# danilodjor/fault-tolerant-llm-training

Measured on AMD Instinct MI355X. Metric: tokens/sec/GPU seq-len 2048 DP at 1/2/4/8 MI355X; checkpoint save wall-clock (s), higher is better.
Workload: dtype bf16; 1 GPU; model=llama3-8b, global_batch=1, seq_len=2048, parallelism=dp1

## Files before the change

csrc/kernels/embedding.hip:

```cpp
#include "torch_utils.h"

#include <algorithm>

namespace {

__global__ __launch_bounds__(256) void emb_fwd_kernel(const int64_t* __restrict__ tok,
                                                      const char* __restrict__ w,
                                                      char* __restrict__ out, int T, int row_bytes) {
  const int row = blockIdx.x;
  const int64_t t = tok[row];
  const uint4* src = reinterpret_cast<const uint4*>(w + t * (long)row_bytes);
  uint4* dst = reinterpret_cast<uint4*>(out + (long)row * row_bytes);
  for (int c = threadIdx.x; c < row_bytes / 16; c += blockDim.x) dst[c] = src[c];
}

constexpr int SORT_NT = 1024, SORT_W = SORT_NT / 64, SORT_BITS = 6, SORT_BINS = 1 << SORT_BITS;

__global__ __launch_bounds__(SORT_NT) void tok_sort_kernel(const int64_t* __restrict__ tok, int T, int passes,
                                                           int* __restrict__ keys, int* __restrict__ vals) {
  __shared__ int hist[SORT_BINS];
  __shared__ int start[SORT_BINS];
  __shared__ int rbase[SORT_BINS];
  __shared__ int wcnt[SORT_W][SORT_BINS];
  const int tid = threadIdx.x, lane = tid & 63, wid = tid >> 6;
// ... 96 lines not shown
                                                         float* __restrict__ part, int nparts) {
  __shared__ float red[4];
  const int lane = threadIdx.x & 63, wid = threadIdx.x >> 6;
  float sq = 0.f;
  for (int wave = blockIdx.x * 4 + wid; wave < T; wave += gridDim.x * 4) {
    const int t = sorted_tok[wave];
    if (wave > 0 && sorted_tok[wave - 1] == t) continue;
    int end = wave + 1;
    while (end < T && sorted_tok[end] == t) ++end;
    typename E::T* dst = dw + t * (long)D;
    for (int c = lane * 8; c < D; c += 64 * 8) {
      float acc[8] = {0, 0, 0, 0, 0, 0, 0, 0};
      for (int k = wave; k < end; ++k) {
        float x[8];
        ld8<E>(dy + perm[k] * (long)D + c, x);
#pragma unroll
        for (int j = 0; j < 8; ++j) acc[j] += x[j];
      }
      const P8<E> r = pk8<E>(acc);
      *reinterpret_cast<uint4*>(dst + c) = r.v[0];
      if constexpr (!E::is16) *reinterpret_cast<uint4*>(dst + c + 4) = r.v[1];
      float st[8];
      unp8<E>(r, st);
#pragma unroll
      for (int j = 0; j < 8; ++j) sq = fmaf(st[j], st[j], sq);
    }
  }
  const float tot = block_sum<256>(sq, red);
  if (threadIdx.x == 0) part[blockIdx.x] = tot;
  for (long i = blockIdx.x + (long)gridDim.x * (1 + threadIdx.x); i < nparts; i += (long)gridDim.x * 256)
    part[i] = 0.f;
}

}

at::Tensor embedding_fwd(const at::Tensor& tokens, const at::Tensor& weight) {
  FT_CHECK_CUDA(weight);
  FT_CHECK_MODEL_DTYPE(weight);
  FT_CHECK_CONTIG(weight);
  FT_CHECK_CONTIG(tokens);
  TORCH_CHECK(tokens.scalar_type() == at::kLong, "embedding: tokens must be int64");
  const int D = weight.size(1);
  TORCH_CHECK(D % 8 == 0, "embedding: dim must be a multiple of 8");
  const int T = tokens.numel();
  const at::DeviceGuard guard(weight.device());
  auto sizes = tokens.sizes().vec();
  sizes.push_back(D);
  auto out = at::empty(sizes, weight.options());
  if (T > 0)
    hipLaunchKernelGGL(emb_fwd_kernel, dim3(T), dim3(256), 0, ft_stream(), cptr<int64_t>(tokens),
                       cptr<char>(weight), mptr<char>(out), T, (int)(D * weight.element_size()));
  FT_LAUNCH_CHECK();
  return out;
}

void embedding_bwd_(const at::Tensor& dy, const at::Tensor& tokens, const at::Tensor& dw,
                    bool accumulate, const std::optional<at::Tensor>& part) {
  FT_CHECK_CUDA(dy);
  FT_CHECK_MODEL_DTYPE(dy);
  TORCH_CHECK(dy.scalar_type() == dw.scalar_type(), "embedding_bwd: dtype mismatch");
  FT_CHECK_CONTIG(dy);
  FT_CHECK_CONTIG(dw);
  const int D = dw.size(1);
  const int T = tokens.numel();
  TORCH_CHECK(dy.numel() == (long)T * D, "embedding_bwd: shape mismatch");
  const at::DeviceGuard guard(dw.device());
  TORCH_CHECK(tokens.scalar_type() == at::kLong, "embedding_bwd: tokens must be int64");
  const long V = dw.size(0);
  TORCH_CHECK(V >= 1 && V < (1L << 30), "embedding_bwd: vocabulary size out of range");
  int bits = 1;
  while ((1L << bits) < V) ++bits;
  const int passes = (bits + SORT_BITS - 1) / SORT_BITS;
  auto flat = tokens.reshape({-1}).contiguous();
  if (!accumulate) FT_HIP_CHECK(hipMemsetAsync(dw.data_ptr(), 0, dw.nbytes(), ft_stream()));
  if (T > 0) {
    auto kv = at::empty({4, (long)T}, tokens.options().dtype(at::kInt));
    int* keys = mptr<int>(kv);
    int* vals = keys + 2L * T;
    hipLaunchKernelGGL(tok_sort_kernel, dim3(1), dim3(SORT_NT), 0, ft_stream(), cptr<int64_t>(flat), T, passes,
                       keys, vals);
    FT_LAUNCH_CHECK();
    const long fin = (long)((passes - 1) & 1) * T;
    const int blocks = (T * 64 + 255) / 256;
    const bool sq = part.has_value() && part->defined();
    if (sq) {
      TORCH_CHECK(!accumulate, "embedding_bwd: norm partials need a fresh gradient");
      FT_CHECK_F32((*part));
      FT_CHECK_CONTIG((*part));
      const int np = (int)part->numel();
      const int g = std::max(1, std::min({blocks, 256, np}));
      FT_DISPATCH_E(dy.scalar_type(),
                    hipLaunchKernelGGL(emb_bwd_sq_kernel<E>, dim3(g), dim3(256), 0, ft_stream(), keys + fin,
                                       vals + fin, cptr<typename E::T>(dy), mptr<typename E::T>(dw), T, D,
                                       mptr<float>(*part), np));
    } else {
      FT_DISPATCH_E(dy.scalar_type(),
                    hipLaunchKernelGGL(emb_bwd_kernel<E>, dim3(blocks), dim3(256), 0, ft_stream(), keys + fin,
                                       vals + fin, cptr<typename E::T>(dy), mptr<typename E::T>(dw), T, D,
                                       accumulate));
    }
  } else if (part.has_value() && part->defined()) {
    part->zero_();
  }
  FT_LAUNCH_CHECK();
}

TORCH_LIBRARY_FRAGMENT(ftamd, m) {
  m.def("embedding_fwd(Tensor tokens, Tensor weight) -> Tensor", &embedding_fwd);
  m.def("embedding_bwd_(Tensor dy, Tensor tokens, Tensor(a!) dw, bool accumulate, Tensor(b!)? part=None) -> ()",
        &embedding_bwd_);
}
```

csrc/kernels/optim.hip:

```cpp
#include "torch_utils.h"

#include <vector>

#include <cstdlib>

namespace {

typedef unsigned int u32x4_t __attribute__((ext_vector_type(4)));

template <bool NT>
__device__ __forceinline__ uint4 ld16(const void* p) {
  if constexpr (NT) {
    const u32x4_t v = __builtin_nontemporal_load(reinterpret_cast<const u32x4_t*>(p));
    return make_uint4(v.x, v.y, v.z, v.w);
  } else {
    return *reinterpret_cast<const uint4*>(p);
  }
}

template <bool NT>
__device__ __forceinline__ void st16(void* p, uint4 v) {
  if constexpr (NT) {
    const u32x4_t w = {v.x, v.y, v.z, v.w};
    __builtin_nontemporal_store(w, reinterpret_cast<u32x4_t*>(p));
  } else {
    *reinterpret_cast<uint4*>(p) = v;
  }
}

template <class E, bool NT>
struct V8 {
  __device__ static void load(const typename E::T* p, float* f) {
    P8<E> r;
    r.v[0] = ld16<NT>(p);
    if constexpr (!E::is16) r.v[1] = ld16<NT>(p + 4);
    unp8<E>(r, f);
  }
  __device__ static void store(typename E::T* p, const float* f) {
    const P8<E> r = pk8<E>(f);
    st16<NT>(p, r.v[0]);
    if constexpr (!E::is16) st16<NT>(p + 4, r.v[1]);
  }
};

bool stream_nt() { return true; }

constexpr int NORM_BLOCKS = 2048;

template <class G, bool NT>
__global__ __launch_bounds__(256) void sumsq_kernel(const typename G::T* __restrict__ g, long n8,
                                                    float* __restrict__ partial) {
  float s = 0.f;
  for (long i = blockIdx.x * 256L + threadIdx.x; i < n8; i += (long)gridDim.x * 256) {
    float x[8];
    V8<G, NT>::load(g + i * 8, x);
#pragma unroll
    for (int j = 0; j < 8; ++j) s += x[j] * x[j];
  }
  __shared__ float red[4];
  s = block_sum<256>(s, red);
  if (threadIdx.x == 0) partial[blockIdx.x] = s;
}

__global__ __launch_bounds__(1024) void norm_finish_kernel(const float* __restrict__ partial,
                                                           int np, float extra_sumsq_scale,
                                                           float max_norm,
                                                           float* __restrict__ stats) {
  float s = 0.f;
  const int n4 = np >> 2;
  const float4* p4 = reinterpret_cast<const float4*>(partial);
  if ((reinterpret_cast<uintptr_t>(partial) & 15) == 0) {
    for (int i = threadIdx.x; i < n4; i += 1024) {
      const float4 v = p4[i];
      s += (v.x + v.y) + (v.z + v.w);
    }
    for (int i = 4 * n4 + threadIdx.x; i < np; i += 1024) s += partial[i];
  } else {
    for (int i = threadIdx.x; i < np; i += 1024) s += partial[i];
  }
  __shared__ float red[16];
  s = block_sum<1024>(s, red);
  if (threadIdx.x == 0) {
    const float norm = sqrtf(s * extra_sumsq_scale);
    stats[0] = norm;
    const bool bad = !isfinite(norm);
    stats[1] = (max_norm > 0.f && !bad) ? fminf(1.f, max_norm / (norm + 1e-6f)) : 1.f;
    stats[2] = (bad || stats[2] != 0.f) ? 1.f : 0.f;
  }
}

template <class P, class S, bool NT>
__global__ __launch_bounds__(256) void adamw_kernel(typename P::T* __restrict__ p,
                                                    const typename P::T* __restrict__ g,
                                                    typename S::T* __restrict__ m,
                                                    typename S::T* __restrict__ v,
                                                    long n8, float lr, float beta1, float beta2,
                                                    float eps, float wd, float inv_bc1,
                                                    float inv_sqrt_bc2,
                                                    const float* __restrict__ stats,
                                                    const float* __restrict__ hyper, int exact) {
  if (stats[2] != 0.f) return;
  if (hyper != nullptr) {
    lr = hyper[0];
    inv_bc1 = hyper[1];
    inv_sqrt_bc2 = hyper[2];
  }
  const float coef = stats[1];
  const float decay = 1.f - lr * wd;
  const float step = lr * inv_bc1;
  for (long i = blockIdx.x * 256L + threadIdx.x; i < n8; i += (long)gridDim.x * 256) {
    float pf[8], gf[8], mf[8], vf[8];
    V8<P, NT>::load(p + i * 8, pf);
    V8<P, NT>::load(g + i * 8, gf);
    V8<S, NT>::load(m + i * 8, mf);
    V8<S, NT>::load(v + i * 8, vf);
#pragma unroll
    for (int j = 0; j < 8; ++j) {
      const float gj = gf[j] * coef;
      pf[j] *= decay;
      mf[j] += (gj - mf[j]) * (1.f - beta1);
      vf[j] = vf[j] * beta2 + (1.f - beta2) * gj * gj;
      if (exact) {
        const float denom = sqrtf(vf[j]) * inv_sqrt_bc2 + eps;
        pf[j] -= step * mf[j] / denom;
      } else {
        const float denom = fast_sqrt(vf[j]) * inv_sqrt_bc2 + eps;
        pf[j] -= step * mf[j] * fast_rcp(denom);
      }
    }
    V8<P, NT>::store(p + i * 8, pf);
    V8<S, NT>::store(m + i * 8, mf);
    V8<S, NT>::store(v + i * 8, vf);
  }
}

int stream_grid(long n8) {
  long g = (n8 + 255) / 256;
  return (int)std::max(1L, std::min(g, 65535L));
}

void launch_sumsq(const at::Tensor& grad, long n8, int nb, float* partial) {
  const bool nt = stream_nt();
  FT_DISPATCH_E(grad.scalar_type(), {
    if (nt)
      hipLaunchKernelGGL((sumsq_kernel<E, true>), dim3(nb), dim3(256), 0, ft_stream(),
                         cptr<typename E::T>(grad), n8, partial);
    else
      hipLaunchKernelGGL((sumsq_kernel<E, false>), dim3(nb), dim3(256), 0, ft_stream(),
                         cptr<typename E::T>(grad), n8, partial);
  });
}

}

void grad_norm_(const at::Tensor& grad, const at::Tensor& stats, double max_norm) {
  FT_CHECK_CUDA(grad);
  FT_CHECK_CONTIG(grad);
  FT_CHECK_F32(stats);
  TORCH_CHECK(grad.numel() % 8 == 0, "grad_norm: numel must be a multiple of 8");
  const at::DeviceGuard guard(grad.device());
  const long n8 = grad.numel() / 8;
  const int nb = std::max(1, std::min(NORM_BLOCKS, (int)((n8 + 255) / 256)));
  auto partial = at::empty({nb}, grad.options().dtype(at::kFloat));
  launch_sumsq(grad, n8, nb, mptr<float>(partial));
  FT_LAUNCH_CHECK();
  hipLaunchKernelGGL(norm_finish_kernel, dim3(1), dim3(1024), 0, ft_stream(), cptr<float>(partial), nb,
// ... 26 lines not shown
  const float bc1 = 1.f - (float)std::pow(beta1, (double)step);
  const float bc2 = 1.f - (float)std::pow(beta2, (double)step);
  const float inv_bc1 = 1.f / bc1, inv_sqrt_bc2 = 1.f / std::sqrt(bc2);
  int nb = stream_grid(n8);
  if (max_blocks > 0) nb = (int)std::max(1L, std::min((n8 + 255) / 256, (long)max_blocks));
  const dim3 grid(nb), block(256);
  const bool nt = stream_nt();
  TORCH_CHECK(m.scalar_type() == p.scalar_type() || m.scalar_type() == at::kFloat,
              "adamw: optimizer states must have the parameter dtype or fp32");
  const int exact = (int)ft_exact_math() || p.scalar_type() == at::kFloat;
  auto go = [&](auto ptag, auto stag) {
    using P = decltype(ptag);
    using S = decltype(stag);
    using PT = typename P::T;
    using ST = typename S::T;
    if (nt)
      hipLaunchKernelGGL((adamw_kernel<P, S, true>), grid, block, 0, ft_stream(), mptr<PT>(p),
                         cptr<PT>(g), mptr<ST>(m), mptr<ST>(v), n8, (float)lr, (float)beta1,
                         (float)beta2, (float)eps, (float)wd, inv_bc1, inv_sqrt_bc2,
                         cptr<float>(stats), hp, exact);
    else
      hipLaunchKernelGGL((adamw_kernel<P, S, false>), grid, block, 0, ft_stream(), mptr<PT>(p),
                         cptr<PT>(g), mptr<ST>(m), mptr<ST>(v), n8, (float)lr, (float)beta1,
                         (float)beta2, (float)eps, (float)wd, inv_bc1, inv_sqrt_bc2,
                         cptr<float>(stats), hp, exact);
  };
  FT_DISPATCH_E(p.scalar_type(), {
    if (m.scalar_type() == at::kFloat) go(E{}, EF32{});
    else go(E{}, E{});
  });
  FT_LAUNCH_CHECK();
}

void sumsq_into_(const at::Tensor& grad, const at::Tensor& partial) {
  FT_CHECK_CUDA(grad);
  FT_CHECK_CONTIG(grad);
  FT_CHECK_F32(partial);
  FT_CHECK_CONTIG(partial);
  TORCH_CHECK(grad.numel() % 8 == 0, "sumsq_into: numel must be a multiple of 8");
  TORCH_CHECK(partial.numel() >= 1 && partial.numel() <= 65535, "sumsq_into: bad partial size");
  const at::DeviceGuard guard(grad.device());
  const long n8 = grad.numel() / 8;
  const int nb = (int)partial.numel();
  launch_sumsq(grad, n8, nb, mptr<float>(partial));
  FT_LAUNCH_CHECK();
}

void norm_finish_(const at::Tensor& partial, const at::Tensor& stats, double max_norm) {
  FT_CHECK_CUDA(partial);
  FT_CHECK_F32(partial);
  FT_CHECK_F32(stats);
  const at::DeviceGuard guard(partial.device());
  hipLaunchKernelGGL(norm_finish_kernel, dim3(1), dim3(1024), 0, ft_stream(), cptr<float>(partial),
                     (int)partial.numel(), 1.f, (float)max_norm, mptr<float>(stats));
  FT_LAUNCH_CHECK();
}

int64_t cu_masked_stream(int64_t stride, int64_t phase) {
  TORCH_CHECK(stride >= 1 && phase >= 0 && phase < stride, "cu_masked_stream: 0 <= phase < stride");
  int dev = 0, ncu = 0;
  FT_HIP_CHECK(hipGetDevice(&dev));
  FT_HIP_CHECK(hipDeviceGetAttribute(&ncu, hipDeviceAttributeMultiprocessorCount, dev));
  std::vector<uint32_t> mask((ncu + 31) / 32, 0u);
  for (int c = (int)phase; c < ncu; c += (int)stride) mask[c / 32] |= 1u << (c % 32);
  hipStream_t st = nullptr;
  FT_HIP_CHECK(hipExtStreamCreateWithCUMask(&st, (uint32_t)mask.size(), mask.data()));
  return reinterpret_cast<int64_t>(st);
}

TORCH_LIBRARY_FRAGMENT(ftamd, m) {
  m.def("cu_masked_stream(int stride, int phase=0) -> int", &cu_masked_stream);
  m.def("sumsq_into_(Tensor grad, Tensor(a!) partial) -> ()", &sumsq_into_);
  m.def("norm_finish_(Tensor partial, Tensor(a!) stats, float max_norm) -> ()", &norm_finish_);
  m.def("grad_norm_(Tensor grad, Tensor(a!) stats, float max_norm) -> ()", &grad_norm_);
  m.def(
      "adamw_(Tensor(a!) p, Tensor g, Tensor(b!) m, Tensor(c!) v, Tensor stats, float lr, float "
      "beta1, float beta2, float eps, float wd, int step, int max_blocks=0, Tensor? hyper=None) -> ()",
      &adamw_);
}
```

fault_tolerant_llm_training_amd/ops/functional.py:

```python
from __future__ import annotations

import collections
import functools
import os
from typing import Optional

import torch
import torch.nn.functional as F

from .._native import kernels, native
from .grad_sink import GradSink

IGNORE_INDEX = -100

_BLAS_ONLY = os.environ.get("FT_GEMM_BLAS", "0") == "1"
_W4_FWD = True
_W4_BWD = os.environ.get("FT_W4_BWD", "1") != "0"
_W4_DTYPES = (torch.bfloat16, torch.float16)
_F32_MFMA = os.environ.get("FT_F32_MFMA", "1") != "0"


def set_f32_mfma(on: bool) -> None:
    global _F32_MFMA
    _F32_MFMA = bool(on)


def f32_route(M: int, N: int, K: int, a_t: bool, b_t: bool, *ts) -> bool:
    if _BLAS_ONLY or not _F32_MFMA or not all(t.is_cuda and t.dtype == torch.float32 for t in ts):
        return False
    return K % 32 == 0 and K > 0 and (not a_t or M % 4 == 0) and (not b_t or N % 4 == 0) and all(
        t.shape[-1] % 4 == 0 for t in ts)
_W4_MIN_TILES = 128
_W4_SHORT_K = 1024
_W4_DEEP_K = 4096
_W4_SMALL = os.environ.get("FT_W4_SMALL", "1") != "0"
_W4_SMALL_WGS = 16


def set_w4_small(on: bool) -> None:
    global _W4_SMALL
    _W4_SMALL = bool(on)


# ... 217 lines not shown


class EmbeddingFn(torch.autograd.Function):
    @staticmethod
    def forward(ctx, tokens, weight, sink):
        ctx.sink = sink
        ctx.vocab = weight.shape[0]
        ctx.save_for_backward(tokens)
        ctx.wshape = weight.shape
        if native(weight):
            return kernels().embedding_fwd(tokens.contiguous(), weight)
        return F.embedding(tokens, weight)

    @staticmethod
    def backward(ctx, dy):
        (tokens,) = ctx.saved_tensors
        sink = ctx.sink
        dy = dy.contiguous()
        if sink is not None and sink.gather is not None:
            if sink.defer:
                sink.stash.append((tokens.reshape(-1), dy.reshape(-1, dy.shape[-1])))
                return None, None, None
            if sink.stash:
                tokens = torch.cat([t for t, _ in sink.stash] + [tokens.reshape(-1)])
                dy = torch.cat([g for _, g in sink.stash] + [dy.reshape(-1, dy.shape[-1])])
                sink.stash = []
            tokens, dy = sink.gather(tokens, dy)
        if native(dy):
            if sink is None:
                dw = torch.zeros(ctx.wshape, dtype=dy.dtype, device=dy.device)
                kernels().embedding_bwd_(dy, tokens.contiguous(), dw, False)
                return None, dw, None
            part = sink.part if (sink.part is not None and not sink.accumulate) else None
            kernels().embedding_bwd_(dy, tokens.contiguous(), sink.buf, sink.accumulate, part)
            if part is not None:
                sink.sq_done = True
            sink.ready()
            return None, None, None
        dw = torch.zeros(ctx.wshape, dtype=torch.float32, device=dy.device)
        if dy.is_cuda:
            dw.index_put_((tokens.reshape(-1),), dy.reshape(-1, ctx.wshape[1]).float(), accumulate=True)
        else:
            dw.index_add_(0, tokens.reshape(-1), dy.reshape(-1, ctx.wshape[1]).float())
        return None, _write_weight_grad(sink, dw.to(dy.dtype)), None


def embedding(tokens, weight, sink=None):
    return EmbeddingFn.apply(tokens, weight, sink)


def norm_reference(x: torch.Tensor, w: torch.Tensor, eps: float, layernorm: bool) -> torch.Tensor:
    xf = x.float()
    if layernorm:
        xf = xf - xf.mean(-1, keepdim=True)
    n = xf * torch.rsqrt(xf.pow(2).mean(-1, keepdim=True) + eps)
    return n.type_as(x) * w


class NormFn(torch.autograd.Function):
    @staticmethod
    def forward(ctx, x, weight, sink, eps, layernorm):
        ctx.sink, ctx.eps, ctx.ln = sink, eps, layernorm
        if native(x):
            xc = x.contiguous()
            y, rstd, mean = kernels().norm_fwd(xc, weight, eps, layernorm)
            ctx.save_for_backward(xc, weight, rstd, mean)
            return y
# ... 360 lines not shown
```

fault_tolerant_llm_training_amd/ops/grad_sink.py:

```python
from __future__ import annotations

from typing import Callable, Optional

import torch


class GradSink:
    __slots__ = ("buf", "start", "end", "accumulate", "hook", "name", "gather", "defer", "stash", "part", "sq_done")

    def __init__(self, buf: torch.Tensor, start: int = 0, end: int = 0, name: str = ""):
        self.buf = buf
        self.start = start
        self.end = end
        self.accumulate = False
        self.hook: Optional[Callable[["GradSink"], None]] = None
        self.name = name
        self.gather: Optional[Callable] = None
        self.defer = False
        self.stash: list = []
        self.part: Optional[torch.Tensor] = None
        self.sq_done = False

    def ready(self) -> None:
        if self.hook is not None:
            self.hook(self)

    def mm(self, a: torch.Tensor, b: torch.Tensor) -> None:
        out = self.buf.view(a.shape[0], b.shape[1])
        if self.accumulate:
            out.addmm_(a, b)
        else:
            torch.mm(a, b, out=out)
        self.ready()

    def set_(self, g: torch.Tensor) -> None:
        if self.accumulate:
            self.buf.add_(g.view_as(self.buf))
        else:
            self.buf.copy_(g.view_as(self.buf))
        self.ready()


def sink_of(p: torch.Tensor) -> Optional[GradSink]:
    return getattr(p, "_ft_sink", None)
```

fault_tolerant_llm_training_amd/optim/adamw.py:

```python
from __future__ import annotations

import math
from typing import List, Optional, Tuple

import torch
import torch.distributed as dist

from .._native import kernels, native
from ..models.flat import FlatParamSpace


class NonFiniteGradError(RuntimeError):
    pass


class ParamGate:

    def __init__(self):
        self.entries: List[list] = []

    def add(self, lo: int, hi: int, handle) -> None:
        self.entries.append([lo, hi, handle])

    def wait(self, lo: int, hi: int) -> None:
        if not self.entries:
            return
        cur = None
        for e in self.entries:
            h = e[2]
            if h is None or e[1] <= lo or e[0] >= hi:
                continue
            if isinstance(h, torch.cuda.Event):
                if cur is None:
                    cur = torch.cuda.current_stream()
                cur.wait_event(h)
            else:
                h.wait()
            e[2] = None
        self.entries = [e for e in self.entries if e[2] is not None]

    def wait_all(self) -> None:
        if self.entries:
# ... 6 lines not shown
    def __init__(self, params, flat: FlatParamSpace, lr: float = 1e-3, betas=(0.9, 0.999),
                 eps: float = 1e-8, weight_decay: float = 1e-2, state_dtype: Optional[torch.dtype] = None,
                 max_grad_norm: float = 0.0, fused: bool = True, reducer=None):
        params = list(params)
        defaults = dict(lr=lr, betas=betas, eps=eps, weight_decay=weight_decay, amsgrad=False,
                        maximize=False, foreach=None, capturable=False, differentiable=False,
                        fused=fused, decoupled_weight_decay=True)
        super().__init__(params, defaults)
        self.flat = flat
        self.reducer = reducer
        self.zero1 = reducer is not None and reducer.mode == "zero1"
        sd = state_dtype or flat.dtype
        n = reducer.shard_numel if self.zero1 else flat.numel
        self.exp_avg = torch.zeros(n, dtype=sd, device=flat.device)
        self.exp_avg_sq = torch.zeros(n, dtype=sd, device=flat.device)
        self.step_count = 0
        self.max_grad_norm = float(max_grad_norm)
        self.stats = torch.zeros(3, dtype=torch.float32, device=flat.device)
        self._pin = flat.device.type == "cuda"
        self._ring = [torch.zeros(3, dtype=torch.float32, pin_memory=self._pin) for _ in range(self.RING)]
        self._ring_events = [None] * self.RING
        self._ring_steps = [-1] * self.RING
        self._checked_step = 0
        self._stats_event = None
        self._stats_step = -1
        self.gate = ParamGate()
        self.graph_mode = False
        self.hyper = torch.zeros(3, dtype=torch.float32, device=flat.device)
        self._hyper_ring = [torch.zeros(3, dtype=torch.float32, pin_memory=self._pin) for _ in range(16)]
        self._hyper_i = 0
        self.overlap_blocks = 0
        name_of = {id(p): n for n, p in flat.param_objs.items()}
        self._index_slots = [flat.slots[name_of[id(p)]] for p in params]

    def clip_grad_norm_(self, max_norm: Optional[float] = None) -> torch.Tensor:
        if max_norm is not None:
            self.max_grad_norm = float(max_norm)
        return self.stats[0]

    def _stream_ctx(self):
        r = self.reducer
        if r is not None and r.overlap:
            return torch.cuda.stream(r.side)
        import contextlib

        return contextlib.nullcontext()

    def _hyper(self):
        grp = self.param_groups[0]
        b1, b2 = grp["betas"]
        return float(grp["lr"]), b1, b2, grp["eps"], grp["weight_decay"]

    def stage_hyper(self, step: int) -> None:
        import numpy as np

        lr, b1, b2, _eps, _wd = self._hyper()
        bc1 = np.float32(1.0) - np.float32(b1 ** step)
        bc2 = np.float32(1.0) - np.float32(b2 ** step)
        h = self._hyper_ring[self._hyper_i % len(self._hyper_ring)]
        self._hyper_i += 1
        h.copy_(torch.from_numpy(np.array([np.float32(lr), np.float32(1.0) / bc1,
                                           np.float32(1.0) / np.sqrt(bc2)], dtype=np.float32)))
        self.hyper.copy_(h, non_blocking=True)

    def _update(self, p, g, m, v, lr, b1, b2, eps, wd, max_blocks: int = 0):
        if native(p):
            kernels().adamw_(p, g, m, v, self.stats, lr, b1, b2, eps, wd, self.step_count, max_blocks,
                             self.hyper if self.graph_mode else None)
        else:
            _adamw_reference(p, g, m, v, self.stats, lr, b1, b2, eps, wd, self.step_count)

    @torch.no_grad()
    def step(self, closure=None):
        self.step_count += 1
        lr, b1, b2, eps, wd = self._hyper()
        f = self.flat
        r = self.reducer
        cuda = f.params.is_cuda
        if r is None:
            if cuda:
                from ..ops.functional import join_dw_stream

                join_dw_stream()
            if native(f.grads):
                kernels().grad_norm_(f.grads, self.stats, self.max_grad_norm)
            else:
                gd = f.grads.double() if f.grads.dtype == torch.float64 else f.grads.float()
                _norm_reference(gd.pow(2).sum().reshape(1), self.stats, self.max_grad_norm)
            self._update(f.params, f.grads, self.exp_avg, self.exp_avg_sq, lr, b1, b2, eps, wd)
            self._publish_stats()
            return None
        if r.overlap:
            r.side.wait_stream(torch.cuda.current_stream())
        with self._stream_ctx():
            total = r.global_sumsq()
            if cuda:
                kernels().norm_finish_(total, self.stats, self.max_grad_norm)
            else:
                _norm_reference(total.sum().reshape(1), self.stats, self.max_grad_norm)
            if not self.graph_mode:
                self._publish_stats()
            for b in sorted(r.buckets, key=lambda b: b.lo):
                slo, shi = r.state_range(b)
                self._update(r.param_for_update(b), r.grad_for_update(b), self.exp_avg[slo:shi],
                             self.exp_avg_sq[slo:shi], lr, b1, b2, eps, wd,
                             self.overlap_blocks if r.overlap else 0)
                if self.zero1 and r.dry_comm:
                    pass
                elif self.zero1 and r.single_stream and r.overlap:
                    dist.all_gather_into_tensor(f.params[b.lo : b.hi], r.param_shard(b), group=r.group)
                    b.agevent.record()
                    self.gate.add(b.lo, b.hi, b.agevent)
                elif self.zero1:
                    work = dist.all_gather_into_tensor(f.params[b.lo : b.hi], r.param_shard(b),
                                                       group=r.group, async_op=True)
                    if r.overlap:
                        self.gate.add(b.lo, b.hi, work)
                    else:
                        work.wait()
                elif r.overlap:
                    b.event.record()
                    self.gate.add(b.lo, b.hi, b.event)
        return None

    def _publish_stats(self):
        i = self.step_count % self.RING
        h = self._ring[i]
        if self.stats.is_cuda:
            h.copy_(self.stats, non_blocking=True)
            ev = self._ring_events[i]
            if ev is None:
                ev = self._ring_events[i] = torch.cuda.Event()
            ev.record()
            self._stats_event = ev
        else:
            h.copy_(self.stats)
        self._ring_steps[i] = self.step_count
        self._stats_step = self.step_count

# ... 18 lines not shown
    def first_nonfinite(self, upto: Optional[int] = None, block: bool = True) -> Optional[int]:
        upto = self.step_count if upto is None else min(int(upto), self.step_count)
        if upto <= self._checked_step:
            return None
        st = self._step_stats(upto, block)
        if st is None:
            return None
        if not st[2]:
            self._checked_step = upto
            return None
        for k in range(max(self._checked_step + 1, self.step_count - self.RING + 1), upto):
            sk = self._step_stats(k, True)
            if sk is not None and sk[2]:
                return k
        return upto

    def last_norm(self) -> Optional[float]:
        st = self._step_stats(self.step_count, True) if self.step_count > 0 else None
        return None if st is None else st[0]

    def check_finite(self, block: bool = False) -> Optional[float]:
        if self.step_count == 0:
            return None
        bad = self.first_nonfinite(block=block)
        if bad is not None:
            raise NonFiniteGradError(nonfinite_message(bad))
        st = self._step_stats(self.step_count, block)
        return None if st is None else st[0]

    @torch.no_grad()
    def reset_nonfinite(self) -> None:
        self.stats.zero_()
        self._checked_step = self.step_count

    def rollback_steps(self, k: int) -> None:
        if k <= 0:
            return
        self.step_count -= k
        self._checked_step = min(self._checked_step, self.step_count)
        for i in range(self.RING):
            if self._ring_steps[i] > self.step_count:
                self._ring_steps[i] = -1

    def zero_grad(self, set_to_none: bool = True):
        return None

    def shard_pieces(self) -> List[Tuple[int, int, int]]:
        r = self.reducer
        return [(b.lo + r.rank * b.shard_len, b.shard_lo, b.shard_len) for b in r.buckets]

    @torch.no_grad()
    def gather_full_state(self, out_m: torch.Tensor, out_v: torch.Tensor) -> None:
        r = self.reducer
        for b in r.buckets:
            slo, shi = r.state_range(b)
            dist.all_gather_into_tensor(out_m[b.lo : b.hi], self.exp_avg[slo:shi], group=r.group)
            dist.all_gather_into_tensor(out_v[b.lo : b.hi], self.exp_avg_sq[slo:shi], group=r.group)

    def state_dict(self, exp_avg: Optional[torch.Tensor] = None, exp_avg_sq: Optional[torch.Tensor] = None):
        if self.zero1 and exp_avg is None:
            raise RuntimeError("ZeRO-1 optimizer state is sharded: pass full-layout moments")
        M = self.exp_avg if exp_avg is None else exp_avg
        V = self.exp_avg_sq if exp_avg_sq is None else exp_avg_sq
        state = {}
        for i, s in enumerate(self._index_slots):
            state[i] = {
# ... 4 lines not shown
        groups = []
        idx = 0
        for g in self.param_groups:
            gg = {k: v for k, v in g.items() if k != "params"}
            gg["params"] = list(range(idx, idx + len(g["params"])))
            idx += len(g["params"])
            groups.append(gg)
        return {"state": state, "param_groups": groups}

    @torch.no_grad()
    def load_state_dict(self, sd):
        from ..ckpt.state import _flat_source

        st = sd["state"]
        slots_by_idx = {i: s for i, s in enumerate(self._index_slots)}
        numel = self.flat.numel
        for key, buf in (("exp_avg", self.exp_avg), ("exp_avg_sq", self.exp_avg_sq)):
            tensors = {i: st[i][key] for i in slots_by_idx if i in st}
            src = None
            if len(tensors) == len(slots_by_idx):
                src = _flat_source(tensors, slots_by_idx, numel, buf.dtype)
            if src is None:
                src = torch.zeros(numel, dtype=buf.dtype)
                for i, t in tensors.items():
                    s = slots_by_idx[i]
                    src[s.offset : s.offset + s.numel].view(s.shape).copy_(t)
            from ..ckpt.restore import h2d

            if self.zero1:
                for flo, slo, n in self.shard_pieces():
                    h2d(buf[slo : slo + n], src[flo : flo + n])
            else:
                h2d(buf, src)
        steps = {int(float(st[i]["step"])) for i in slots_by_idx if i in st}
        if steps:
            self.step_count = max(steps)
        for g, sg in zip(self.param_groups, sd["param_groups"]):
            for k, v in sg.items():
                if k != "params":
                    g[k] = v

    def moments(self):
        return self.exp_avg, self.exp_avg_sq


def nonfinite_message(step: int) -> str:
    return (f"The total norm of order 2.0 for gradients from `parameters` is non-finite at optimizer step {step}, "
            "so it cannot be clipped (update skipped).")


def _norm_reference(sumsq: torch.Tensor, stats: torch.Tensor, max_norm: float) -> None:
    norm = float(sumsq.sqrt())
    bad = not math.isfinite(norm)
    coef = 1.0 if (max_norm <= 0 or bad) else min(1.0, max_norm / (norm + 1e-6))
    sticky = bad or float(stats[2]) != 0.0
    stats.copy_(torch.tensor([norm, coef, 1.0 if sticky else 0.0]))


def _adamw_reference(p, g, m, v, stats, lr, b1, b2, eps, wd, step):
    if stats[2].item() != 0:
        return
    coef = stats[1].item()
    md = torch.float64 if p.dtype == torch.float64 else torch.float32
    gf = g.to(md) * coef
    pf = p.to(md) * (1 - lr * wd)
    mf = m.to(md)
# ... 11 lines not shown
```

fault_tolerant_llm_training_amd/parallel/ddp.py:

```python
from __future__ import annotations

import os
from typing import List, Optional

import torch
import torch.distributed as dist

from .._native import kernels, native
from ..models.flat import FlatParamSpace
from ..ops.grad_sink import GradSink

MODES = ("local", "allreduce", "zero1")
LOCAL_BUCKET_MB = 64.0
DP_BUCKET_MB = 256.0
PARTIALS_PER_BUCKET = 512
SUMSQ_AT_END = False


def set_sumsq_at_end(on: bool) -> None:
    global SUMSQ_AT_END
    SUMSQ_AT_END = bool(on)


FUSED_SUMSQ = True
# ... 361 lines not shown

    def finish(self) -> None:
        if self.cuda:
            from ..ops.functional import join_dw_stream

            join_dw_stream()
        while self._next < len(self.buckets):
            b = self.buckets[self._next]
            self._next += 1
            self._launch(b)
        if self._pending_sumsq:
            with torch.cuda.stream(self.side):
                for b in self._pending_sumsq:
                    self._sumsq(self.grad_for_update(b), b)
            self._pending_sumsq = []
        if not self.overlap:
            for b in self.buckets:
                if b.work is not None:
                    b.work.wait()
                    b.work = None
                    self._post(b)
                self._sumsq(self.grad_for_update(b), b)
        for b in self.buckets:
            b.filled = 0
            b.launched = False
        self._next = 0
        self.gathered = False

    @torch.no_grad()
    def poison_and_complete(self, tokens_shape=None, dim: int = 0) -> None:
        self.sync = True
        nan = float("nan")
        poisoned = False
        for b in self.buckets[self._next:]:
            self.flat.grads[b.lo : b.hi].fill_(nan)
            poisoned = True
        while self._next < len(self.buckets) and not self.buckets[self._next].sparse:
            b = self.buckets[self._next]
            self._next += 1
            self._launch(b)
        if self.sparse_embedding and not self.gathered:
            T = 1
            for s_ in tokens_shape or (1,):
                T *= int(s_)
            tok = torch.zeros(T, dtype=torch.long, device=self.flat.device)
            dy = torch.full((T, dim), nan, dtype=self.flat.dtype, device=self.flat.device)
            self._gather_rows(tok, dy)
            es = self.emb_sink
            self.flat.grads[es.start : es.end].fill_(nan)
            poisoned = True
        del poisoned
        self.finish()

    def global_sumsq(self) -> torch.Tensor:
        if self.mode != "zero1":
            return self.partials
        if self.cuda:
            torch.sum(self.partials, dim=0, keepdim=True, out=self.sumsq_total)
        else:
            self.sumsq_total.copy_(self.partials.sum().reshape(1))
        if not self.dry_comm:
            dist.all_reduce(self.sumsq_total, op=dist.ReduceOp.SUM, group=self.group)
        return self.sumsq_total

    @torch.no_grad()
    def broadcast_params(self, src: int = 0) -> None:
# ... 10 lines not shown
```

Baseline: 20750 tokens/s (whole job, sum over GPUs).

## Track touched embedding rows to skip dense grad clears and cold-row Adam work

Adds per-row state for the token embedding. Backward now zeros only the rows touched in the previous step instead of memsetting the whole gradient, and records which rows got gradients this step. A row-aware AdamW kernel runs the full moment update only on rows with a gradient or nonzero moments, and applies just weight decay to the cold rows. This cuts memory traffic over the large embedding table for Llama3-8B, in exchange for more state bookkeeping, refresh passes after restore or nonfinite steps, and a risk of correctness bugs in the row state.

```diff
diff --git a/csrc/kernels/embedding.hip b/csrc/kernels/embedding.hip
--- a/csrc/kernels/embedding.hip
+++ b/csrc/kernels/embedding.hip
@@ -152,6 +152,34 @@
     part[i] = 0.f;
 }
 
+constexpr unsigned ROW_WARM = 1u, ROW_GRAD = 2u;
+
+__global__ __launch_bounds__(256) void emb_rows_clear_kernel(const int* __restrict__ rows,
+                                                             const int* __restrict__ count, int cap,
+                                                             char* __restrict__ dw, uint8_t* __restrict__ state,
+                                                             int V, int row_bytes) {
+  const int n = min(*count, cap);
+  for (int i = blockIdx.x; i < n; i += gridDim.x) {
+    const int t = rows[i];
+    if (t < 0 || t >= V) continue;
+    uint4* dst = reinterpret_cast<uint4*>(dw + t * (long)row_bytes);
+    for (int c = threadIdx.x; c < row_bytes / 16; c += blockDim.x) dst[c] = make_uint4(0, 0, 0, 0);
+    if (threadIdx.x == 0) state[t] &= (uint8_t)~ROW_GRAD;
+  }
+}
+
+__global__ __launch_bounds__(256) void emb_rows_record_kernel(const int* __restrict__ sorted_tok, int T, int V,
+                                                              int* __restrict__ rows, int* __restrict__ count,
+                                                              uint8_t* __restrict__ state) {
+  const int i = blockIdx.x * blockDim.x + threadIdx.x;
+  if (i == 0) *count = T;
+  if (i >= T) return;
+  const int t = sorted_tok[i];
+  const bool head = (i == 0 || sorted_tok[i - 1] != t) && t >= 0 && t < V;
+  rows[i] = head ? t : -1;
+  if (head) state[t] |= (uint8_t)(ROW_WARM | ROW_GRAD);
+}
+
 }
 
 at::Tensor embedding_fwd(const at::Tensor& tokens, const at::Tensor& weight) {
@@ -174,8 +202,18 @@
   return out;
 }
 
-void embedding_bwd_(const at::Tensor& dy, const at::Tensor& tokens, const at::Tensor& dw,
-                    bool accumulate, const std::optional<at::Tensor>& part) {
+namespace {
+
+struct RowMeta {
+  uint8_t* state;
+  int* rows;
+  int* count;
+  int cap;
+  bool reset;
+};
+
+void embedding_bwd_impl(const at::Tensor& dy, const at::Tensor& tokens, const at::Tensor& dw, bool accumulate,
+                        const std::optional<at::Tensor>& part, const RowMeta* meta) {
   FT_CHECK_CUDA(dy);
   FT_CHECK_MODEL_DTYPE(dy);
   TORCH_CHECK(dy.scalar_type() == dw.scalar_type(), "embedding_bwd: dtype mismatch");
@@ -192,15 +230,26 @@
   while ((1L << bits) < V) ++bits;
   const int passes = (bits + SORT_BITS - 1) / SORT_BITS;
   auto flat = tokens.reshape({-1}).contiguous();
-  if (!accumulate) FT_HIP_CHECK(hipMemsetAsync(dw.data_ptr(), 0, dw.nbytes(), ft_stream()));
+  const int row_bytes = (int)(D * dw.element_size());
+  if (meta != nullptr && !meta->reset) {
+    TORCH_CHECK(row_bytes % 16 == 0, "embedding_bwd_rows: rows must be whole 16-B vectors");
+    hipLaunchKernelGGL(emb_rows_clear_kernel, dim3(std::max(1, T)), dim3(256), 0, ft_stream(), meta->rows,
+                       meta->count, meta->cap, mptr<char>(dw), meta->state, (int)V, row_bytes);
+    FT_LAUNCH_CHECK();
+  } else if (!accumulate) {
+    FT_HIP_CHECK(hipMemsetAsync(dw.data_ptr(), 0, dw.nbytes(), ft_stream()));
+  }
+  const int* sorted = nullptr;
+  at::Tensor kv;
   if (T > 0) {
-    auto kv = at::empty({4, (long)T}, tokens.options().dtype(at::kInt));
+    kv = at::empty({4, (long)T}, tokens.options().dtype(at::kInt));
     int* keys = mptr<int>(kv);
     int* vals = keys + 2L * T;
     hipLaunchKernelGGL(tok_sort_kernel, dim3(1), dim3(SORT_NT), 0, ft_stream(), cptr<int64_t>(flat), T, passes,
                        keys, vals);
     FT_LAUNCH_CHECK();
     const long fin = (long)((passes - 1) & 1) * T;
+    sorted = keys + fin;
     const int blocks = (T * 64 + 255) / 256;
     const bool sq = part.has_value() && part->defined();
     if (sq) {
@@ -223,10 +272,42 @@
     part->zero_();
   }
   FT_LAUNCH_CHECK();
+  if (meta != nullptr) {
+    hipLaunchKernelGGL(emb_rows_record_kernel, dim3(std::max(1, (T + 255) / 256)), dim3(256), 0, ft_stream(),
+                       sorted, T, (int)V, meta->rows, meta->count, meta->state);
+    FT_LAUNCH_CHECK();
+  }
+}
+
+}
+
+void embedding_bwd_(const at::Tensor& dy, const at::Tensor& tokens, const at::Tensor& dw,
+                    bool accumulate, const std::optional<at::Tensor>& part) {
+  embedding_bwd_impl(dy, tokens, dw, accumulate, part, nullptr);
+}
+
+void embedding_bwd_rows_(const at::Tensor& dy, const at::Tensor& tokens, const at::Tensor& dw,
+                         const std::optional<at::Tensor>& part, const at::Tensor& state, const at::Tensor& rows,
+                         const at::Tensor& count, bool reset) {
+  FT_CHECK_CUDA(dw);
+  for (const at::Tensor* t : {&state, &rows, &count})
+    TORCH_CHECK(t->is_cuda() && t->device() == dw.device() && t->is_contiguous(),
+                "embedding_bwd_rows: metadata must be contiguous on dw's device");
+  TORCH_CHECK(state.scalar_type() == at::kByte && state.numel() == dw.size(0),
+              "embedding_bwd_rows: state must be uint8 [V]");
+  TORCH_CHECK(rows.scalar_type() == at::kInt && count.scalar_type() == at::kInt && count.numel() == 1,
+              "embedding_bwd_rows: rows / count must be int32");
+  TORCH_CHECK(rows.numel() >= tokens.numel(), "embedding_bwd_rows: the row list is shorter than the token count");
+  const RowMeta meta{mptr<uint8_t>(state), mptr<int>(rows), mptr<int>(count), (int)rows.numel(), reset};
+  embedding_bwd_impl(dy, tokens, dw, false, part, &meta);
 }
 
 TORCH_LIBRARY_FRAGMENT(ftamd, m) {
   m.def("embedding_fwd(Tensor tokens, Tensor weight) -> Tensor", &embedding_fwd);
   m.def("embedding_bwd_(Tensor dy, Tensor tokens, Tensor(a!) dw, bool accumulate, Tensor(b!)? part=None) -> ()",
         &embedding_bwd_);
-}
+  m.def(
+      "embedding_bwd_rows_(Tensor dy, Tensor tokens, Tensor(a!) dw, Tensor(b!)? part, Tensor(c!) state, "
+      "Tensor(d!) rows, Tensor(e!) count, bool reset) -> ()",
+      &embedding_bwd_rows_);
+}
diff --git a/csrc/kernels/optim.hip b/csrc/kernels/optim.hip
--- a/csrc/kernels/optim.hip
+++ b/csrc/kernels/optim.hip
@@ -35,6 +35,12 @@
     r.v[0] = ld16<NT>(p);
     if constexpr (!E::is16) r.v[1] = ld16<NT>(p + 4);
     unp8<E>(r, f);
+  }
+  __device__ static P8<E> loadp(const typename E::T* p) {
+    P8<E> r;
+    r.v[0] = ld16<NT>(p);
+    if constexpr (!E::is16) r.v[1] = ld16<NT>(p + 4);
+    return r;
   }
   __device__ static void store(typename E::T* p, const float* f) {
     const P8<E> r = pk8<E>(f);
@@ -89,6 +95,41 @@
   }
 }
 
+struct AdamwK {
+  float coef, decay, step, beta1, beta2, eps, inv_sqrt_bc2;
+  int exact;
+};
+
+__device__ __forceinline__ AdamwK adamw_scalars(float lr, float beta1, float beta2, float eps, float wd,
+                                                float inv_bc1, float inv_sqrt_bc2,
+                                                const float* __restrict__ stats,
+                                                const float* __restrict__ hyper, int exact) {
+  if (hyper != nullptr) {
+    lr = hyper[0];
+    inv_bc1 = hyper[1];
+    inv_sqrt_bc2 = hyper[2];
+  }
+  return AdamwK{stats[1], 1.f - lr * wd, lr * inv_bc1, beta1, beta2, eps, inv_sqrt_bc2, exact};
+}
+
+__device__ __forceinline__ void adamw_update8(float* pf, const float* gf, float* mf, float* vf,
+                                              const AdamwK& k) {
+#pragma unroll
+  for (int j = 0; j < 8; ++j) {
+    const float gj = gf[j] * k.coef;
+    pf[j] *= k.decay;
+    mf[j] += (gj - mf[j]) * (1.f - k.beta1);
+    vf[j] = fmaf(k.beta2, vf[j], (1.f - k.beta2) * gj * gj);
+    if (k.exact) {
+      const float denom = sqrtf(vf[j]) * k.inv_sqrt_bc2 + k.eps;
+      pf[j] -= k.step * mf[j] / denom;
+    } else {
+      const float denom = fast_sqrt(vf[j]) * k.inv_sqrt_bc2 + k.eps;
+      pf[j] -= k.step * mf[j] * fast_rcp(denom);
+    }
+  }
+}
+
 template <class P, class S, bool NT>
 __global__ __launch_bounds__(256) void adamw_kernel(typename P::T* __restrict__ p,
                                                     const typename P::T* __restrict__ g,
@@ -100,38 +141,83 @@
                                                     const float* __restrict__ stats,
                                                     const float* __restrict__ hyper, int exact) {
   if (stats[2] != 0.f) return;
-  if (hyper != nullptr) {
-    lr = hyper[0];
-    inv_bc1 = hyper[1];
-    inv_sqrt_bc2 = hyper[2];
-  }
-  const float coef = stats[1];
-  const float decay = 1.f - lr * wd;
-  const float step = lr * inv_bc1;
+  const AdamwK k = adamw_scalars(lr, beta1, beta2, eps, wd, inv_bc1, inv_sqrt_bc2, stats, hyper, exact);
   for (long i = blockIdx.x * 256L + threadIdx.x; i < n8; i += (long)gridDim.x * 256) {
     float pf[8], gf[8], mf[8], vf[8];
     V8<P, NT>::load(p + i * 8, pf);
     V8<P, NT>::load(g + i * 8, gf);
     V8<S, NT>::load(m + i * 8, mf);
     V8<S, NT>::load(v + i * 8, vf);
-#pragma unroll
-    for (int j = 0; j < 8; ++j) {
-      const float gj = gf[j] * coef;
-      pf[j] *= decay;
-      mf[j] += (gj - mf[j]) * (1.f - beta1);
-      vf[j] = vf[j] * beta2 + (1.f - beta2) * gj * gj;
-      if (exact) {
-        const float denom = sqrtf(vf[j]) * inv_sqrt_bc2 + eps;
-        pf[j] -= step * mf[j] / denom;
-      } else {
-        const float denom = fast_sqrt(vf[j]) * inv_sqrt_bc2 + eps;
-        pf[j] -= step * mf[j] * fast_rcp(denom);
-      }
-    }
+    adamw_update8(pf, gf, mf, vf, k);
     V8<P, NT>::store(p + i * 8, pf);
     V8<S, NT>::store(m + i * 8, mf);
     V8<S, NT>::store(v + i * 8, vf);
   }
+}
+
+constexpr unsigned ROW_WARM = 1u, ROW_GRAD = 2u;
+
+template <class P, class S, bool NT>
+__global__ __launch_bounds__(256) void adamw_rows_kernel(typename P::T* __restrict__ p,
+                                                         const typename P::T* __restrict__ g,
+                                                         typename S::T* __restrict__ m,
+                                                         typename S::T* __restrict__ v,
+                                                         uint8_t* __restrict__ state, int V, int D8,
+                                                         float lr, float beta1, float beta2, float eps,
+                                                         float wd, float inv_bc1, float inv_sqrt_bc2,
+                                                         const float* __restrict__ stats,
+                                                         const float* __restrict__ hyper, int exact) {
+  if (stats[2] != 0.f) return;
+  const AdamwK k = adamw_scalars(lr, beta1, beta2, eps, wd, inv_bc1, inv_sqrt_bc2, stats, hyper, exact);
+  for (int row = blockIdx.x; row < V; row += gridDim.x) {
+    const unsigned st = state[row];
+    __syncthreads();
+    const long base = (long)row * D8;
+    if (st & (ROW_GRAD | ROW_WARM)) {
+      const bool has_g = (st & ROW_GRAD) != 0;
+      P8<P> gzero = zp8<P>();
+      pin8<P>(gzero);
+      for (int c = threadIdx.x; c < D8; c += 256) {
+        const long i = (base + c) * 8;
+        float pf[8], gf[8], mf[8], vf[8];
+        V8<P, NT>::load(p + i, pf);
+        P8<P> gp = gzero;
+        if (has_g) gp = V8<P, NT>::loadp(g + i);
+        unp8<P>(gp, gf);
+        V8<S, NT>::load(m + i, mf);
+        V8<S, NT>::load(v + i, vf);
+        adamw_update8(pf, gf, mf, vf, k);
+        V8<P, NT>::store(p + i, pf);
+        V8<S, NT>::store(m + i, mf);
+        V8<S, NT>::store(v + i, vf);
+      }
+      if (has_g && threadIdx.x == 0) state[row] = (uint8_t)ROW_WARM;
+    } else {
+      for (int c0 = threadIdx.x; c0 < D8; c0 += 512) {
+        const int c1 = c0 + 256;
+        const bool two = c1 < D8;
+        const long i0 = (base + c0) * 8, i1 = (base + (two ? c1 : c0)) * 8;
+        float pf[2][8];
+        V8<P, NT>::load(p + i0, pf[0]);
+        if (two) V8<P, NT>::load(p + i1, pf[1]);
+#pragma unroll
+        for (int j = 0; j < 8; ++j) pf[0][j] *= k.decay;
+        V8<P, NT>::store(p + i0, pf[0]);
+        if (two) {
+#pragma unroll
+          for (int j = 0; j < 8; ++j) pf[1][j] *= k.decay;
+          V8<P, NT>::store(p + i1, pf[1]);
+        }
+      }
+    }
+  }
+}
+
+__global__ __launch_bounds__(256) void adamw_rows_consume_kernel(uint8_t* __restrict__ state, int V,
+                                                                 const float* __restrict__ stats) {
+  if (stats[2] != 0.f) return;
+  const int row = blockIdx.x * 256 + threadIdx.x;
+  if (row < V && (state[row] & ROW_GRAD)) state[row] = (uint8_t)ROW_WARM;
 }
 
 int stream_grid(long n8) {
@@ -224,6 +310,73 @@
   FT_LAUNCH_CHECK();
 }
 
+void adamw_rows_(const at::Tensor& p, const at::Tensor& g, const at::Tensor& m, const at::Tensor& v,
+                 const at::Tensor& state, const at::Tensor& stats, double lr, double beta1, double beta2,
+                 double eps, double wd, int64_t step, const std::optional<at::Tensor>& hyper) {
+  const float* hp = nullptr;
+  if (hyper.has_value() && hyper->defined()) {
+    FT_CHECK_F32((*hyper));
+    TORCH_CHECK(hyper->is_cuda() && hyper->numel() >= 3, "adamw_rows: hyper must be a device fp32[3]");
+    hp = cptr<float>(*hyper);
+  }
+  FT_CHECK_CUDA(p);
+  FT_CHECK_CONTIG(p);
+  FT_CHECK_CONTIG(g);
+  FT_CHECK_CONTIG(m);
+  FT_CHECK_CONTIG(v);
+  FT_CHECK_CONTIG(state);
+  FT_CHECK_F32(stats);
+  TORCH_CHECK(p.dim() == 2 && p.sizes() == g.sizes() && p.sizes() == m.sizes() && p.sizes() == v.sizes(),
+              "adamw_rows: p, g, m, v must be [V, D]");
+  TORCH_CHECK(p.size(1) % 8 == 0 && p.size(0) >= 1 && p.size(0) < (1L << 31) && p.size(1) < (1L << 31),
+              "adamw_rows: D must be a multiple of 8");
+  TORCH_CHECK(state.is_cuda() && state.scalar_type() == at::kByte && state.numel() == p.size(0),
+              "adamw_rows: state must be a device uint8 [V]");
+  TORCH_CHECK(p.scalar_type() == g.scalar_type() && m.scalar_type() == v.scalar_type(),
+              "adamw_rows: dtype mismatch");
+  TORCH_CHECK(m.scalar_type() == p.scalar_type() || m.scalar_type() == at::kFloat,
+              "adamw_rows: optimizer states must have the parameter dtype or fp32");
+  for (const at::Tensor* t : {&p, &g, &m, &v})
+    TORCH_CHECK((reinterpret_cast<uintptr_t>(t->data_ptr()) & 15) == 0, "adamw_rows: buffers must be 16-B aligned");
+  TORCH_CHECK(eps > 0, "adamw_rows: eps must be positive (the cold-row update relies on a finite 1/eps)");
+  const at::DeviceGuard guard(p.device());
+  const int V = (int)p.size(0), D8 = (int)(p.size(1) / 8);
+  if (p.scalar_type() == at::kHalf) {
+    adamw_(p.view({-1}), g.view({-1}), m.view({-1}), v.view({-1}), stats, lr, beta1, beta2, eps, wd, step, 0, hyper);
+    hipLaunchKernelGGL(adamw_rows_consume_kernel, dim3((V + 255) / 256), dim3(256), 0, ft_stream(),
+                       mptr<uint8_t>(state), V, cptr<float>(stats));
+    FT_LAUNCH_CHECK();
+    return;
+  }
+  const float bc1 = 1.f - (float)std::pow(beta1, (double)step);
+  const float bc2 = 1.f - (float)std::pow(beta2, (double)step);
+  const float inv_bc1 = 1.f / bc1, inv_sqrt_bc2 = 1.f / std::sqrt(bc2);
+  const dim3 grid(V), block(256);
+  const bool nt = stream_nt();
+  const int exact = (int)ft_exact_math() || p.scalar_type() == at::kFloat;
+  auto go = [&](auto ptag, auto stag) {
+    using P = decltype(ptag);
+    using S = decltype(stag);
+    using PT = typename P::T;
+    using ST = typename S::T;
+    if (nt)
+      hipLaunchKernelGGL((adamw_rows_kernel<P, S, true>), grid, block, 0, ft_stream(), mptr<PT>(p),
+                         cptr<PT>(g), mptr<ST>(m), mptr<ST>(v), mptr<uint8_t>(state), V, D8, (float)lr,
+                         (float)beta1, (float)beta2, (float)eps, (float)wd, inv_bc1, inv_sqrt_bc2,
+                         cptr<float>(stats), hp, exact);
+    else
+      hipLaunchKernelGGL((adamw_rows_kernel<P, S, false>), grid, block, 0, ft_stream(), mptr<PT>(p),
+                         cptr<PT>(g), mptr<ST>(m), mptr<ST>(v), mptr<uint8_t>(state), V, D8, (float)lr,
+                         (float)beta1, (float)beta2, (float)eps, (float)wd, inv_bc1, inv_sqrt_bc2,
+                         cptr<float>(stats), hp, exact);
+  };
+  FT_DISPATCH_E(p.scalar_type(), {
+    if (m.scalar_type() == at::kFloat) go(E{}, EF32{});
+    else go(E{}, E{});
+  });
+  FT_LAUNCH_CHECK();
+}
+
 void sumsq_into_(const at::Tensor& grad, const at::Tensor& partial) {
   FT_CHECK_CUDA(grad);
   FT_CHECK_CONTIG(grad);
@@ -269,4 +422,8 @@
       "adamw_(Tensor(a!) p, Tensor g, Tensor(b!) m, Tensor(c!) v, Tensor stats, float lr, float "
       "beta1, float beta2, float eps, float wd, int step, int max_blocks=0, Tensor? hyper=None) -> ()",
       &adamw_);
-}
+  m.def(
+      "adamw_rows_(Tensor(a!) p, Tensor g, Tensor(b!) m, Tensor(c!) v, Tensor(d!) state, Tensor stats, float "
+      "lr, float beta1, float beta2, float eps, float wd, int step, Tensor? hyper=None) -> ()",
+      &adamw_rows_);
+}
diff --git a/fault_tolerant_llm_training_amd/ops/functional.py b/fault_tolerant_llm_training_amd/ops/functional.py
--- a/fault_tolerant_llm_training_amd/ops/functional.py
+++ b/fault_tolerant_llm_training_amd/ops/functional.py
@@ -9,6 +9,7 @@
 import torch.nn.functional as F
 
 from .._native import kernels, native
+from . import grad_sink as _grad_sink
 from .grad_sink import GradSink
 
 IGNORE_INDEX = -100
@@ -292,7 +293,17 @@
                 kernels().embedding_bwd_(dy, tokens.contiguous(), dw, False)
                 return None, dw, None
             part = sink.part if (sink.part is not None and not sink.accumulate) else None
-            kernels().embedding_bwd_(dy, tokens.contiguous(), sink.buf, sink.accumulate, part)
+            rows = sink.rows
+            if rows is not None and _grad_sink.EMB_ROWS and not sink.accumulate and sink.gather is None:
+                T = tokens.numel()
+                reset = rows.begin_fresh(T)
+                kernels().embedding_bwd_rows_(dy, tokens.contiguous(), sink.buf, part, rows.state, rows.rows,
+                                              rows.count, reset)
+                rows.valid = rows.pending = True
+            else:
+                if rows is not None:
+                    rows.dense_backward(tokens)
+                kernels().embedding_bwd_(dy, tokens.contiguous(), sink.buf, sink.accumulate, part)
             if part is not None:
                 sink.sq_done = True
             sink.ready()
diff --git a/fault_tolerant_llm_training_amd/ops/grad_sink.py b/fault_tolerant_llm_training_amd/ops/grad_sink.py
--- a/fault_tolerant_llm_training_amd/ops/grad_sink.py
+++ b/fault_tolerant_llm_training_amd/ops/grad_sink.py
@@ -1,12 +1,66 @@
 from __future__ import annotations
 
+import os
 from typing import Callable, Optional
 
 import torch
 
+EMB_ROWS = os.environ.get("FT_EMB_ROWS", "1") == "1"
+
+
+def set_emb_rows(on: bool) -> None:
+    global EMB_ROWS
+    EMB_ROWS = bool(on)
+
+
+ROW_WARM = 1
+ROW_GRAD = 2
+
+
+class EmbRows:
+
+    def __init__(self, vocab: int, device):
+        self.state = torch.zeros(vocab, dtype=torch.uint8, device=device)
+        self.rows = torch.full((1,), -1, dtype=torch.int32, device=device)
+        self.count = torch.zeros(1, dtype=torch.int32, device=device)
+        self.valid = False
+        self.pending = False
+        self.warm_stale = True
+
+    def invalidate(self) -> None:
+        self.valid = False
+        self.pending = False
+        self.warm_stale = True
+
+    def dense_backward(self, tokens: torch.Tensor) -> None:
+        self.valid = False
+        self.pending = False
+        self.state.index_fill_(0, tokens.reshape(-1), ROW_WARM)
+
+    def begin_fresh(self, T: int) -> bool:
+        reset = not self.valid
+        if self.rows.numel() < T:
+            self.rows = torch.full((T,), -1, dtype=torch.int32, device=self.state.device)
+            reset = True
+        if reset:
+            self.state.bitwise_and_(ROW_WARM)
+        return reset
+
+    def mark_all_warm(self) -> None:
+        self.state.bitwise_or_(ROW_WARM)
+        self.warm_stale = False
+
+    @torch.no_grad()
+    def refresh_warm(self, m: torch.Tensor, v: torch.Tensor) -> None:
+        bits = {2: torch.int16, 4: torch.int32}[m.element_size()]
+        warm = (m.view(bits) != 0).any(1) | (v.view(bits) != 0).any(1)
+        self.state.bitwise_and_(ROW_GRAD).bitwise_or_(warm.to(torch.uint8))
+        self.warm_stale = False
+
+
 
 class GradSink:
-    __slots__ = ("buf", "start", "end", "accumulate", "hook", "name", "gather", "defer", "stash", "part", "sq_done")
+    __slots__ = ("buf", "start", "end", "accumulate", "hook", "name", "gather", "defer", "stash", "part", "sq_done", "rows")
 
     def __init__(self, buf: torch.Tensor, start: int = 0, end: int = 0, name: str = ""):
         self.buf = buf
@@ -20,6 +74,7 @@
         self.stash: list = []
         self.part: Optional[torch.Tensor] = None
         self.sq_done = False
+        self.rows: Optional[EmbRows] = None
 
     def ready(self) -> None:
         if self.hook is not None:
diff --git a/fault_tolerant_llm_training_amd/optim/adamw.py b/fault_tolerant_llm_training_amd/optim/adamw.py
--- a/fault_tolerant_llm_training_amd/optim/adamw.py
+++ b/fault_tolerant_llm_training_amd/optim/adamw.py
@@ -8,6 +8,8 @@
 
 from .._native import kernels, native
 from ..models.flat import FlatParamSpace
+from ..ops import grad_sink as _grad_sink
+from ..ops.grad_sink import EmbRows
 
 
 class NonFiniteGradError(RuntimeError):
@@ -80,6 +82,43 @@
         self.overlap_blocks = 0
         name_of = {id(p): n for n, p in flat.param_objs.items()}
         self._index_slots = [flat.slots[name_of[id(p)]] for p in params]
+        self._emb_rows = None
+        self._emb_bucket = None
+        sink = flat.sinks.get("tok_embeddings.weight")
+        if sink is not None:
+            sink.rows = None
+        if (sink is not None and reducer is not None and reducer.mode == "local" and native(flat.params)
+                and native(self.exp_avg) and sink.buf.dim() == 2 and sink.buf.shape[1] % 8 == 0):
+            for b in reducer.buckets:
+                if b.lo == sink.start and b.hi == sink.end:
+                    self._emb_bucket = b
+                    self._emb_rows = sink.rows = EmbRows(sink.buf.shape[0], flat.device)
+
+    def _row_moments(self):
+        b = self._emb_bucket
+        shape = self.flat.sinks["tok_embeddings.weight"].buf.shape
+        return self.exp_avg[b.lo : b.hi].view(shape), self.exp_avg_sq[b.lo : b.hi].view(shape)
+
+    @torch.no_grad()
+    def refresh_row_state(self) -> None:
+        if self._emb_rows is not None:
+            self._emb_rows.refresh_warm(*self._row_moments())
+
+    def debug_mark_all_rows_warm(self) -> None:
+        if self._emb_rows is not None:
+            self._emb_rows.mark_all_warm()
+
+    def _use_rows(self, b, eps: float) -> bool:
+        rows = self._emb_rows
+        if rows is None or b is not self._emb_bucket or not (_grad_sink.EMB_ROWS and rows.valid and rows.pending):
+            return False
+        if eps <= 0 or self.flat.sinks["tok_embeddings.weight"].accumulate:
+            return False
+        if rows.warm_stale:
+            if torch.cuda.is_current_stream_capturing():
+                return False
+            self.refresh_row_state()
+        return True
 
     def clip_grad_norm_(self, max_norm: Optional[float] = None) -> torch.Tensor:
         if max_norm is not None:
@@ -117,6 +156,15 @@
                              self.hyper if self.graph_mode else None)
         else:
             _adamw_reference(p, g, m, v, self.stats, lr, b1, b2, eps, wd, self.step_count)
+
+    def _update_rows(self, b, lr, b1, b2, eps, wd):
+        rows = self._emb_rows
+        shape = self.flat.sinks["tok_embeddings.weight"].buf.shape
+        m, v = self._row_moments()
+        kernels().adamw_rows_(self.flat.params[b.lo : b.hi].view(shape), self.flat.grads[b.lo : b.hi].view(shape),
+                              m, v, rows.state, self.stats, lr, b1, b2, eps, wd, self.step_count,
+                              self.hyper if self.graph_mode else None)
+        rows.pending = False
 
     @torch.no_grad()
     def step(self, closure=None):
@@ -150,9 +198,12 @@
                 self._publish_stats()
             for b in sorted(r.buckets, key=lambda b: b.lo):
                 slo, shi = r.state_range(b)
-                self._update(r.param_for_update(b), r.grad_for_update(b), self.exp_avg[slo:shi],
-                             self.exp_avg_sq[slo:shi], lr, b1, b2, eps, wd,
-                             self.overlap_blocks if r.overlap else 0)
+                if self._use_rows(b, eps):
+                    self._update_rows(b, lr, b1, b2, eps, wd)
+                else:
+                    self._update(r.param_for_update(b), r.grad_for_update(b), self.exp_avg[slo:shi],
+                                 self.exp_avg_sq[slo:shi], lr, b1, b2, eps, wd,
+                                 self.overlap_blocks if r.overlap else 0)
                 if self.zero1 and r.dry_comm:
                     pass
                 elif self.zero1 and r.single_stream and r.overlap:
@@ -237,6 +288,7 @@
     def reset_nonfinite(self) -> None:
         self.stats.zero_()
         self._checked_step = self.step_count
+        self.refresh_row_state()
 
     def rollback_steps(self, k: int) -> None:
         if k <= 0:
@@ -307,6 +359,7 @@
                     h2d(buf[slo : slo + n], src[flo : flo + n])
             else:
                 h2d(buf, src)
+        self.refresh_row_state()
         steps = {int(float(st[i]["step"])) for i in slots_by_idx if i in st}
         if steps:
             self.step_count = max(steps)
diff --git a/fault_tolerant_llm_training_amd/parallel/ddp.py b/fault_tolerant_llm_training_amd/parallel/ddp.py
--- a/fault_tolerant_llm_training_amd/parallel/ddp.py
+++ b/fault_tolerant_llm_training_amd/parallel/ddp.py
@@ -417,6 +417,9 @@
         self.sync = True
         nan = float("nan")
         poisoned = False
+        emb_sink = self.flat.sinks.get("tok_embeddings.weight")
+        if emb_sink is not None and emb_sink.rows is not None:
+            emb_sink.rows.invalidate()
         for b in self.buckets[self._next:]:
             self.flat.grads[b.lo : b.hi].fill_(nan)
             poisoned = True
```

Measured after the change: 20920 tokens/s (whole job, sum over GPUs), median of 6. Within noise of the previous version (+0.8%).
